# hruffieux/atlasqtl

Hardware: AMD Instinct MI355X
Metric: VB sweeps/sec (higher is better)
Workload: dtype f64; 1 GPU; atlasqtl VB sweep (S1-S22 incl. scheduled ELBO), n=1000 p=50000 q=10000, anneal=(1,2,10) on, horseshoe global-local, sweeps 6-93; n=1000, p=50000, q=10000, q_per_gpu=10000, parallelism=trait-sharded x1, env_overrides=

## Files before the change

atlasqtl_amd/csrc/aq_core_sweep.h:

```cpp
#pragma once
#include <hip/hip_runtime.h>
#include "aq_special.h"
#include "aq_plan_const.h"

typedef double aq_d4 __attribute__((ext_vector_type(4)));

struct AqCoreArgs {
  const double2 *XA;
  const double2 *XU;
  const double *G;
  const double *Gx;
  double *R;
  double *gam;
  double *mu;
  const double *Aarr;
  const double *Barr;
  const double *coef;
  const double *inv2s;
  const double *cst;
  const double *sig2b;
  double *sums;
  double *rowGB;
  double c;
  int p, q;
  int p_pad, q_pad, n_pad, nb, ntile;
  int dmode;
  int mode;
  int nseg;
  int stagger;
  int *done;
  int *errflag;
  int C;
  int xtouch;
  int xhelper;
  double *Pbuf;
  int *pflag;
  double *rnpart;
  const double *mis;
  const double *GK;
  const double *tau, *log_tau;
  const double *sig2_inv_p, *log_sig2_inv_p;
  long long *dbg;
  const double *theta;
  const double *zeta;
  double sqrt_c;
  int c_is_one;
  int mprio;
  int hprio;
};

__device__ __forceinline__ aq_d4 aq_mfma(double a, double b, aq_d4 c) {
  return __builtin_amdgcn_mfma_f64_16x16x4f64(a, b, c, 0, 0, 0);
}
__device__ __forceinline__ void aq_lds_barrier() { asm volatile("s_waitcnt lgkmcnt(0)\n\ts_barrier" ::: "memory"); }
__device__ __forceinline__ int aq_drow(int dmode, int reg, int g) { return (dmode ? 1 : 4) * reg + (dmode ? 4 : 1) * g; }
```

atlasqtl_amd/csrc/aq_core_sweep_la.h:

```cpp
#pragma once
#include <hip/hip_runtime.h>
#include "aq_core_sweep.h"
#include <type_traits>

typedef double aq_v2 __attribute__((ext_vector_type(2)));

__device__ __forceinline__ double aq_row16_sum(double v) {
  auto step = [&](auto ctrl) __attribute__((always_inline)) {
    constexpr int C = decltype(ctrl)::value;
    const int lo = __builtin_amdgcn_update_dpp(0, __double2loint(v), C, 0xf, 0xf, false);
    const int hi = __builtin_amdgcn_update_dpp(0, __double2hiint(v), C, 0xf, 0xf, false);
    v += __hiloint2double(hi, lo);
  };
  step(std::integral_constant<int, 0xB1>{});
  step(std::integral_constant<int, 0x4E>{});
  step(std::integral_constant<int, 0x124>{});
  step(std::integral_constant<int, 0x128>{});
  return v;
}

#ifndef AQ_GLDS_AUX
#define AQ_GLDS_AUX 2
#endif
__device__ __forceinline__ void aq_glds16(const void *gsrc_lane, void *lds_base) {
// ... 206 lines not shown
  }

  constexpr int NTT = 3 * (NT + NT2) + NT3;
  const int nblk_s = a.mode == 1 ? 0 : nblk;
  auto run = [&](auto ntc, auto rolec, auto hook) __attribute__((always_inline)) {
    constexpr int NTC = decltype(ntc)::value;
    constexpr int ROLE = decltype(rolec)::value;
    constexpr bool HI = ROLE == 0;
    constexpr int ST = (NTC + 2) / 3;
    const int my_t0 = part * NTT + (ROLE == 0 ? mw * NT : ROLE == 1 ? 3 * NT + (mw - 3) * NT2 : 3 * (NT + NT2));
    const int slot = ROLE == 2 ? NWM : mw;
    aq_d4 Rr[TT][NTC];
    unsigned long long mb0 = 0, mb1 = 0;
    aq_static_for<TT>([&](auto ttc) __attribute__((always_inline)) {
      constexpr int tt = decltype(ttc)::value;
      const double *Rg = a.R + (size_t)(tile0 + tt) * a.n_pad * 16 + (size_t)(16 * my_t0 + g) * 16 + col;
      aq_static_for<NTC>([&](auto tc) __attribute__((always_inline)) {
        constexpr int t = decltype(tc)::value;
#pragma unroll
        for (int r = 0; r < 4; r++) Rr[tt][t][r] = Rg[(16 * t + 4 * r) * 16];
        if constexpr (MASK) {
          const double *Mg = a.mis + (size_t)tile0 * a.n_pad * 16 + (size_t)(16 * my_t0 + g) * 16 + col;
#pragma unroll
          for (int r = 0; r < 4; r++)
            if (Mg[(16 * t + 4 * r) * 16] != 0.0) { if (t < 16) mb0 |= 1ull << (4 * (t & 15) + r); else mb1 |= 1ull << (4 * (t & 15) + r); }
        }
      });
    });
    auto remask = [&](auto tc) __attribute__((always_inline)) {
      constexpr int t = decltype(tc)::value;
      const unsigned long long mb = t < 16 ? mb0 : mb1;
#pragma unroll
      for (int r = 0; r < 4; r++) Rr[0][t][r] = ((mb >> (4 * (t & 15) + r)) & 1ull) ? Rr[0][t][r] : 0.0;
    };
    const unsigned voff = (unsigned)((my_t0 * 128 + lane) * 16);
    const char *XUb = (const char *)a.XU, *XAb = (const char *)a.XA;
    const long long BLK = (long long)NTT * C * 128 * 16;
    aq_v2 p0, p1, q0, q1, c0, c1, d0, d1;
#ifdef AQ_FORCE_DEEP_DB
#ifdef AQ_FORCE_DEEP_TT2
    constexpr bool DEEP = (NTC >= 4);
#else
    constexpr bool DEEP = (TT == 1) && (NTC >= 4);
#endif
    constexpr int DB = !DEEP ? 1 : AQ_FORCE_DEEP_DB;
#elif defined(AQ_FORCE_DEEP_MASK_DB)
    constexpr bool DEEP = (TT == 1) && (NTC >= 4) && (MASK || true);
    constexpr int DB = !DEEP ? 1 : MASK ? AQ_FORCE_DEEP_MASK_DB : (NT <= 11) ? AQ_DEEP_TT1 : 3;
#else
    constexpr bool DEEP = (TT == 1) && (NTC >= 4) && (!MASK || (SEG && NT <= 11));
    constexpr int DB = !DEEP ? 1 : (!MASK && NT <= 11) ? AQ_DEEP_TT1 : 3;
#endif
    aq_v2 xb[DB][2], ab[DB][2];
    auto dangling = [&](const char *xu0, const char *xa0, auto skip_first) __attribute__((always_inline)) {
      aq_static_for<DB - 1>([&](auto jc) __attribute__((always_inline)) {
        constexpr int j = decltype(jc)::value;
        if constexpr (!(decltype(skip_first)::value && j == 0)) {
          constexpr int kb = (j + 2) / 4, imm = (j - 4 * kb) * 2048;
          AQ_LD2I(xb[j][0], xb[j][1], voff, xu0 + kb * 8192, imm);
        }
        if constexpr (j <= DB - 3) {
          constexpr int kb = (j + 2) / 4, imm = (j - 4 * kb) * 2048;
          AQ_LD2I(ab[j][0], ab[j][1], voff, xa0 + kb * 8192, imm);
        }
      });
    };
    if constexpr (DEEP) {
      dangling(XUb + seg_b0 * BLK, XAb + seg_b0 * BLK, std::false_type{});
    } else {
      AQ_LD2(p0, p1, voff, XUb + seg_b0 * BLK);
      AQ_LD2(c0, c1, voff, XAb + seg_b0 * BLK);
    }
    for (int i = 0; i <= nblk + 1; i++) {
      const bool do_u = i >= 2, do_s = i < nblk_s;
      const double mflag = do_u ? -1.0 : 0.0;
      const int bu = seg_b0 + (i >= 2 ? i - 2 : 0), bs = seg_b0 + (i < nblk ? i : nblk - 1);
      const int nbu = seg_b0 + (i >= 1 ? (i - 1 < nblk ? i - 1 : nblk - 1) : 0), nbs = seg_b0 + (i + 1 < nblk ? i + 1 : nblk - 1);
      tl_mark(i, 0);
      hook(i);
      tl_mark(i, 1);
      if (do_u && (ROLE != 2 || a.mode == 1)) wait_ge(6, i - 1);
      if (ROLE == 1 && a.stagger) wait_ge(8 + (mw - 3), i + 1);
      tl_mark(i, 2);
      double nd[TT][4];
      {
        unsigned zero = 0;
        asm volatile("" : "+v"(zero));
        const int ln = __builtin_amdgcn_mbcnt_hi(~0u, __builtin_amdgcn_mbcnt_lo(~0u, zero));
        const double *dl = &Ldel[bu & 1][(ln >> 4) * NTR + (ln & 15)];
#pragma unroll
        for (int tt = 0; tt < TT; tt++)
#pragma unroll
          for (int s = 0; s < 4; s++) nd[tt][s] = dl[4 * NTR * s + 16 * tt] * mflag;
      }
      aq_d4 acc[TT];
#pragma unroll
      for (int tt = 0; tt < TT; tt++) acc[tt] = (aq_d4){0, 0, 0, 0};
      const char *xu = XUb + __builtin_amdgcn_readfirstlane(bu) * BLK, *xa = XAb + __builtin_amdgcn_readfirstlane(bs) * BLK;
      const char *nxu = XUb + __builtin_amdgcn_readfirstlane(nbu) * BLK, *nxa = XAb + __builtin_amdgcn_readfirstlane(nbs) * BLK;
      if (ROLE != 2 && a.mprio) __builtin_amdgcn_s_setprio(0);
      auto U = [&](auto tc, aq_v2 u0, aq_v2 u1) __attribute__((always_inline)) {
        constexpr int t = decltype(tc)::value;
        aq_static_for<TT>([&](auto ttc) __attribute__((always_inline)) {
          constexpr int tt = decltype(ttc)::value;
          aq_d4 Rt = Rr[tt][t];
          Rt = aq_mfma(u0.x, nd[tt][0], Rt);
          Rt = aq_mfma(u0.y, nd[tt][1], Rt);
          Rt = aq_mfma(u1.x, nd[tt][2], Rt);
          Rt = aq_mfma(u1.y, nd[tt][3], Rt);
          Rr[tt][t] = Rt;
        });
      };
      auto S = [&](auto tc, aq_v2 x0, aq_v2 x1) __attribute__((always_inline)) {
        constexpr int t = decltype(tc)::value;
        aq_static_for<TT>([&](auto ttc) __attribute__((always_inline)) {
          constexpr int tt = decltype(ttc)::value;
          const aq_d4 Rp = Rr[tt][t];
          acc[tt] = aq_mfma(x0.x, Rp[0], acc[tt]);
          acc[tt] = aq_mfma(x0.y, Rp[1], acc[tt]);
          acc[tt] = aq_mfma(x1.x, Rp[2], acc[tt]);
          acc[tt] = aq_mfma(x1.y, Rp[3], acc[tt]);
        });
      };
      if constexpr (DEEP) {
        aq_static_for<NTC>([&](auto tc) __attribute__((always_inline)) {
          constexpr int t = decltype(tc)::value, last = NTC - 1;
          using TP = std::integral_constant<int, (t > 0 ? t - 1 : 0)>;
          if constexpr (t + DB - 1 <= last) {
            constexpr int k = t + DB - 1, kb = (k + 2) / 4, imm = (k - 4 * kb) * 2048;
            AQ_LD2I(xb[k % DB][0], xb[k % DB][1], voff, xu + kb * 8192, imm);
          }
          if constexpr (t + DB - 2 <= last) {
            constexpr int k = t + DB - 2, kb = (k + 2) / 4, imm = (k - 4 * kb) * 2048;
            AQ_LD2I(ab[k % DB][0], ab[k % DB][1], voff, xa + kb * 8192, imm);
          }
          constexpr int issued = aq_req_issued(DB, last, t);
          aq_wait2n<2 * (issued - 1 - aq_req_index(DB, last, 0, t))>(xb[t % DB][0], xb[t % DB][1]);
          U(tc, xb[t % DB][0], xb[t % DB][1]);
          __builtin_amdgcn_sched_barrier(0);
          if constexpr (t >= 1) {
            constexpr int k = t - 1;
            aq_wait2n<2 * (issued - 1 - aq_req_index(DB, last, 1, k))>(ab[k % DB][0], ab[k % DB][1]);
            S(TP{}, ab[k % DB][0], ab[k % DB][1]);
            __builtin_amdgcn_sched_barrier(0);
          }
          if constexpr (MASK) {
            remask(tc);
            __builtin_amdgcn_sched_barrier(0);
          }
          if constexpr (t == last) {
            AQ_LD2I(xb[0][0], xb[0][1], voff, nxu, 0);
            aq_wait2n<2 * (issued - 1 - aq_req_index(DB, last, 1, last) + 1)>(ab[last % DB][0], ab[last % DB][1]);
            S(tc, ab[last % DB][0], ab[last % DB][1]);
            __builtin_amdgcn_sched_barrier(0);
            dangling(nxu, nxa, std::true_type{});
          }
          if constexpr (HI && t + 1 == ST) {
            if (a.stagger) signal(8 + mw, i + 1);
          }
          __builtin_amdgcn_sched_barrier(0);
        });
      } else if constexpr (NTC == 1) {
        using C0 = std::integral_constant<int, 0>;
        AQ_WAIT2(0, p0, p1);
        AQ_WAIT2(0, c0, c1);
        U(C0{}, p0, p1);
        if (HI && a.stagger) signal(8 + mw, i + 1);
        __builtin_amdgcn_sched_barrier(0);
        AQ_LD2(p0, p1, voff, nxu);
        if constexpr (MASK) remask(C0{});
        S(C0{}, c0, c1);
        __builtin_amdgcn_sched_barrier(0);
        AQ_LD2(c0, c1, voff, nxa);
      } else {
        aq_static_for<NTC>([&](auto tc) __attribute__((always_inline)) {
          constexpr int t = decltype(tc)::value;
          constexpr bool even = (t & 1) == 0, last = (t == NTC - 1);
          using TP = std::integral_constant<int, (t > 0 ? t - 1 : 0)>;
          if constexpr (!last) {
            constexpr int kb = (t + 1 + 2) / 4, imm = (t + 1 - 4 * kb) * 2048;
            if constexpr (even) { AQ_LD2I(q0, q1, voff, xu + kb * 8192, imm); }
            else { AQ_LD2I(p0, p1, voff, xu + kb * 8192, imm); }
          }
          if constexpr (t >= 1) {
            constexpr int kc = (t + 2) / 4, immc = (t - 4 * kc) * 2048;
            if constexpr (even) { AQ_LD2I(c0, c1, voff, xa + kc * 8192, immc); }
            else { AQ_LD2I(d0, d1, voff, xa + kc * 8192, immc); }
          }
          if constexpr (t == 0) AQ_WAIT2(4, p0, p1);
          else if constexpr (last && t == 1) AQ_WAIT2(2, q0, q1);
          else if constexpr (last) { if constexpr (even) AQ_WAIT2(4, p0, p1); else AQ_WAIT2(4, q0, q1); }
          else if constexpr (t == 1) { AQ_WAIT2(4, q0, q1); AQ_WAIT2(4, c0, c1); }
          else if constexpr (even) AQ_WAIT2(6, p0, p1);
          else AQ_WAIT2(6, q0, q1);
          if constexpr (even) U(tc, p0, p1); else U(tc, q0, q1);
          __builtin_amdgcn_sched_barrier(0);
          if constexpr (t >= 1) {
            if constexpr (last) { if constexpr (even) AQ_WAIT2(2, d0, d1); else AQ_WAIT2(2, c0, c1); }
            else if constexpr (t >= 2) { if constexpr (even) AQ_WAIT2(4, d0, d1); else AQ_WAIT2(4, c0, c1); }
            if constexpr (even) S(TP{}, d0, d1); else S(TP{}, c0, c1);
            __builtin_amdgcn_sched_barrier(0);
          }
          if constexpr (MASK) {
            remask(tc);
            __builtin_amdgcn_sched_barrier(0);
          }
          if constexpr (last) {
            AQ_LD2(p0, p1, voff, nxu);
            if constexpr (even) { AQ_WAIT2(2, c0, c1); S(tc, c0, c1); }
            else { AQ_WAIT2(2, d0, d1); S(tc, d0, d1); }
            __builtin_amdgcn_sched_barrier(0);
            AQ_LD2(c0, c1, voff, nxa);
          }
          if constexpr (HI && t + 1 == ST) {
            if (a.stagger) signal(8 + mw, i + 1);
          }
          __builtin_amdgcn_sched_barrier(0);
        });
      }
      if (ROLE != 2 && a.mprio) __builtin_amdgcn_s_setprio(2);
      if (do_s) {
        const int ps = bs & 1;
#pragma unroll
        for (int tt = 0; tt < TT; tt++)
#pragma unroll
          for (int r = 0; r < 4; r++) Sp[ps][slot][(4 * r + g) * NTR + 16 * tt + col] = acc[tt][r];
      }
      signal(ROLE == 2 ? 11 : mw, i + 1);
      tl_mark(i, 3);
    }
    if constexpr (DEEP) {
      asm volatile("s_waitcnt vmcnt(0)" ::: "memory");
      asm volatile("" : "+v"(xb[0][0]), "+v"(xb[0][1]), "+v"(ab[0][0]), "+v"(ab[0][1]));
      if constexpr (DB > 1) asm volatile("" : "+v"(xb[DB > 1 ? 1 : 0][0]), "+v"(xb[DB > 1 ? 1 : 0][1]), "+v"(ab[DB > 1 ? 1 : 0][0]), "+v"(ab[DB > 1 ? 1 : 0][1]));
      if constexpr (DB > 2) asm volatile("" : "+v"(xb[DB > 2 ? 2 : 0][0]), "+v"(xb[DB > 2 ? 2 : 0][1]), "+v"(ab[DB > 2 ? 2 : 0][0]), "+v"(ab[DB > 2 ? 2 : 0][1]));
      if constexpr (DB > 3) asm volatile("" : "+v"(xb[DB > 3 ? 3 : 0][0]), "+v"(xb[DB > 3 ? 3 : 0][1]), "+v"(ab[DB > 3 ? 3 : 0][0]), "+v"(ab[DB > 3 ? 3 : 0][1]));
    }
    else
      asm volatile("s_waitcnt vmcnt(0)" : "+v"(p0), "+v"(p1), "+v"(c0), "+v"(c1), "+v"(q0), "+v"(q1), "+v"(d0), "+v"(d1));
    unsigned zero2 = 0;
    asm volatile("" : "+v"(zero2));
    const int ln2 = __builtin_amdgcn_mbcnt_hi(~0u, __builtin_amdgcn_mbcnt_lo(~0u, zero2));
    double *Rout = a.R;
    asm volatile("" : "+s"(Rout));
    aq_static_for<TT>([&](auto ttc) __attribute__((always_inline)) {
      constexpr int tt = decltype(ttc)::value;
      double *Rg = Rout + (size_t)(tile0 + tt) * a.n_pad * 16 + (size_t)(16 * my_t0 + (ln2 >> 4)) * 16 + (ln2 & 15);
      double rn = 0.0;
      aq_static_for<NTC>([&](auto tc) __attribute__((always_inline)) {
        constexpr int t = decltype(tc)::value;
#pragma unroll
        for (int r = 0; r < 4; r++) {
          const double v = Rr[tt][t][r];
          Rg[(16 * t + 4 * r) * 16] = v;
          rn += v * v;
        }
      });
      Lrn[slot * 4 + (ln2 >> 4)][16 * tt + (ln2 & 15)] = rn;
    });
  };
  const auto no_hook = [](int) {};

  bool split_dead = false;
// ... 337 lines not shown
    double sv_g[MASK ? RPG : 1], sv_m[MASK ? RPG : 1], sv_xn[MASK ? RPG : 1], sv_th[MASK ? RPG : 1];
    auto pre_load = [&](int b) __attribute__((always_inline)) {
      const double *gk = gk_block(b);
#pragma unroll
      for (int r = 0; r < RPG; r++) {
        const size_t off = tbase + (size_t)(16 * b + hg + NG * r) * 16;
        const int jj = hg + NG * r;
        pl_g[r] = a.gam[off];
        pl_m[r] = a.mu[off];
        pl_xn[r] = gk[(jj * (jj + 1) / 2 + jj) * 16 + ht];
      }
    };
    auto stage_dma = [&](int b, int par, int b_next) __attribute__((always_inline)) {
#pragma unroll
      for (int r = 0; r < RPG; r++) {
        asm volatile("" : "+v"(pl_g[r]), "+v"(pl_m[r]), "+v"(pl_xn[r]), "+v"(th[r]) : : "memory");
        sv_g[r] = pl_g[r]; sv_m[r] = pl_m[r]; sv_xn[r] = pl_xn[r]; sv_th[r] = th[r];
      }
      gk_dma(b, par);
      if (b_next < seg_b1) { pre_load(b_next); theta_load(b_next); }
    };
    auto stage = [&](int b, int par) __attribute__((always_inline)) {
      double st_G[4], st_Gx[4], st_xn[MASK ? RPG : 1];
      if constexpr (MASK) {
#pragma unroll
        for (int r = 0; r < RPG; r++) { Lm1[par][lane + 64 * r] = sv_g[r] * sv_m[r]; st_xn[r] = sv_xn[r]; }
      } else {
#pragma unroll
        for (int r = 0; r < RPG; r++) Lm1[par][lane + 64 * r] = pg[r] * pm[r];
#pragma unroll
        for (int r = 0; r < 4; r++) {
          st_G[r] = a.G[(size_t)b * 256 + lane + 64 * r];
          const int bx = CXC ? (b + 1 < a.nb ? b + 1 : b) : b;
          st_Gx[r] = a.Gx[(size_t)bx * 256 + lane + 64 * r];
        }
      }
      double ls2r[MASK ? RPG : 1];
      if constexpr (MASK) {
#pragma unroll
        for (int r = 0; r < RPG; r++) {
          const int e = lane + 64 * r;
          const double is2 = a.c * (st_xn[r] + sig2_inv_h) * tau_k;
          const double s2 = aq_recip_pos(is2);
          const double ls2 = -aq_log_pos(is2);
          const double cf = a.c * s2 * tau_k;
          Lcoef[par][e] = cf;
          LK[par][e] = cf * cf * (a.c * 0.5 * is2);
          Ls2[par][e] = s2;
          Lls2[par][e] = ls2;
          Lxn[par][e] = st_xn[r];
          ls2r[r] = ls2;
        }
      }
      auto emitA = [&](int r, double A) __attribute__((always_inline)) {
        const int j = 16 * b + hg + NG * r, e = lane + 64 * r;
        const bool valid = kvalid && j < a.p;
        if constexpr (MASK) {
          LA[par][e] = a.c * ((valid ? A : 0.0) - 0.5 * ls2r[r] + cstna_k);
        } else {
          LA[par][e] = a.c * ((valid ? A : 0.0) + cst_k);
        }
      };
      auto emitZ = [&](int r, double zb, double za) __attribute__((always_inline)) {
        const int j = 16 * b + hg + NG * r, e = lane + 64 * r;
        const bool valid = kvalid && j < a.p;
        LB[par][e] = valid ? zb : 0.0;
        Laa[par][e] = valid ? za : 0.0;
      };
      auto emit2 = [&](int r, double A, double zb, double za) __attribute__((always_inline)) {
        const int j = 16 * b + hg + NG * r, e = lane + 64 * r;
        const bool valid = kvalid && j < a.p;
        LB[par][e] = valid ? zb : 0.0;
        Laa[par][e] = valid ? za : 0.0;
        if constexpr (MASK) LA[par][e] = a.c * ((valid ? A : 0.0) - 0.5 * Lls2[par][e] + cstna_k);
        else LA[par][e] = a.c * ((valid ? A : 0.0) + cst_k);
      };
      double uu[RPG];
      bool inr = true;
#pragma unroll
      for (int r = 0; r < RPG; r++) {
        uu[r] = (MASK ? sv_th[r] : th[r]) + zk;
        inr = inr && fabs(uu[r]) < AQ_PT_R && fabs(a.sqrt_c * uu[r]) < AQ_PT_R;
      }
      {
        constexpr int NC = AQ_PT_DEG + 1, S = AQ_PT_NI, F = NC * S;
        auto locate = [&](double x, double *xloc) __attribute__((always_inline)) {
          const double t = fmin(fabs(x) * (1.0 / AQ_PT_W), AQ_PT_NI * (1.0 - 0x1p-53));
          const int i = (int)t;
          *xloc = fma(2.0, t - (double)i, -1.0);
          return ptab + i;
        };
        {
          double co[2][NC], xl[2];
          auto fetch = [&](int r, auto setc) __attribute__((always_inline)) {
            constexpr int set = decltype(setc)::value;
            aq_lds_cdouble *pp = locate(uu[r], &xl[set]);
#pragma unroll
            for (int k = 0; k < NC; k++) co[set][k] = pp[k * S];
          };
          fetch(0, std::integral_constant<int, 0>{});
          aq_static_for<RPG>([&](auto rc) __attribute__((always_inline)) {
            constexpr int r = decltype(rc)::value, set = r & 1;
            if constexpr (r + 1 < RPG) fetch(r + 1, std::integral_constant<int, (r + 1) & 1>{});
            __builtin_amdgcn_sched_barrier(0);
            double pa = co[set][NC - 1];
#pragma unroll
            for (int k = NC - 2; k >= 0; k--) pa = fma(pa, xl[set], co[set][k]);
            emitA(r, uu[r] < 0.0 ? -pa : pa);
            __builtin_amdgcn_sched_barrier(0);
          });
        }
        {
          double co[2][2 * NC], xl[2];
          auto fetch = [&](int r, auto setc) __attribute__((always_inline)) {
            constexpr int set = decltype(setc)::value;
            aq_lds_cdouble *pp = locate(a.sqrt_c * uu[r], &xl[set]);
#pragma unroll
            for (int k = 0; k < NC; k++) {
              co[set][k] = pp[F + k * S];
              co[set][NC + k] = pp[2 * F + k * S];
            }
          };
          fetch(0, std::integral_constant<int, 0>{});
          aq_static_for<RPG>([&](auto rc) __attribute__((always_inline)) {
            constexpr int r = decltype(rc)::value, set = r & 1;
            if constexpr (r + 1 < RPG) fetch(r + 1, std::integral_constant<int, (r + 1) & 1>{});
            __builtin_amdgcn_sched_barrier(0);
            double pb = co[set][NC - 1], pd = co[set][2 * NC - 1];
#pragma unroll
            for (int k = NC - 2; k >= 0; k--) {
              pb = fma(pb, xl[set], co[set][k]);
              pd = fma(pd, xl[set], co[set][NC + k]);
            }
            const double d = uu[r] < 0.0 ? -pd : pd;
            emitZ(r, pb * inv_sqrt_c, uu[r] - 0.5 * inv_sqrt_c * (pb + d));
            __builtin_amdgcn_sched_barrier(0);
          });
        }
      }
      if (__builtin_expect(!__all(inr), 0)) {
#pragma unroll 1
        for (int r = 0; r < RPG; r++) {
          double ur = uu[0];
#pragma unroll
          for (int k = 1; k < RPG; k++) ur = (r == k) ? uu[k] : ur;
          double A, bM, dM, dummy;
          aq_probit_tab_eval<1>(ur, ptab, &A, &dummy, &dummy);
          aq_probit_tab_eval<2>(a.sqrt_c * ur, ptab, &dummy, &bM, &dM);
          emit2(r, A, bM * inv_sqrt_c, ur - 0.5 * inv_sqrt_c * (bM + dM));
        }
      }
      if constexpr (MASK) {
#ifdef AQ_DIAG_TIME
        const long long t_dma = __builtin_readcyclecounter();
#endif
        asm volatile("s_waitcnt vmcnt(0)" ::: "memory");
#ifdef AQ_DIAG_TIME
        dg_wait += __builtin_readcyclecounter() - t_dma;
#endif
      } else {
#pragma unroll
        for (int r = 0; r < 4; r++) {
          const int e = lane + 64 * r;
          LG[par][(e >> 4) * 32 + (e & 15)] = st_G[r];
          LGx[CXC ? (b + 1) % 3 : par][e] = st_Gx[r];
        }
      }
    };
    double cs0 = 0.0, cs1 = 0.0, cs2 = 0.0, cs3 = 0.0, cs5 = 0.0;
    auto finalize = [&](int b, int par) __attribute__((always_inline)) {
#pragma unroll
      for (int r = 0; r < RPG; r++) {
        const int e = lane + 64 * r, hj = hg + NG * r;
        const double gm = Lgam[par][e], mu = Lmu[par][e];
        const size_t off = tbase + (size_t)(16 * b + hj) * 16;
        if (lead) {
          a.gam[off] = gm;
          a.mu[off] = mu;
        }
        const int j = 16 * b + hj;
        double gb = 0.0;
        if (kvalid && j < a.p) {
          const double be = gm * mu;
          gb = Laa[par][e] + gm * LB[par][e];
          cs0 += gm;
          cs3 += gb;
          if constexpr (MASK) {
            const double s2 = Ls2[par][e];
            const double m2 = (mu * mu + s2) * gm;
            const double xn = Lxn[par][e];
            cs1 += m2;
            cs2 += xn * (m2 - be * be);
            cs5 += gm * Lls2[par][e];
          } else {
            cs1 += (mu * mu + sig2b_k) * gm;
            cs2 += be * be;
          }
        }
        gb = aq_row16_sum(gb);
        if ((ht & 15) == 0 && lead) a.rowGB[(size_t)(tile0 + (ht >> 4)) * a.p_pad + j] = gb;
      }
    };
    auto exchange = [&](int b) __attribute__((always_inline)) {
      const int par = b & 1, kdone = b - seg_b0 + 1;
      if constexpr (WIDE) tl_mark(kdone, 0);
#pragma unroll
      for (int m = 0; m < NWM; m++) wait_ge(m, kdone);
      if constexpr (NT3 > 0) wait_ge(11, kdone);
      if constexpr (WIDE) tl_mark(kdone, 1);
      double own[RPG];
#pragma unroll
      for (int r = 0; r < RPG; r++) {
        const int e = lane + 64 * r;
        double sv = Sp[par][0][e];
#pragma unroll
        for (int ww = 1; ww < NPS; ww++) sv += Sp[par][ww][e];
        own[r] = sv;
      }
      if constexpr (WIDE) split_exchange_wide(b, own, [] {});
      else split_exchange(b, own, [] {});
#pragma unroll
      for (int r = 0; r < RPG; r++) Stot[par][lane + 64 * r] = own[r];
      signal(14, kdone);
    };
    if (a.mode == 1) {
      for (int b = seg_b0; b < seg_b1; b++) {
        const int k = b - seg_b0, par = b & 1;
        if (k >= 2) {
#pragma unroll
          for (int m = 0; m < NWM; m++) wait_ge(m, k + 1);
          if (NT3 > 0) wait_ge(11, k + 1);
        }
#pragma unroll
        for (int r = 0; r < RPG; r++) {
          const int e = lane + 64 * r, hj = hg + NG * r;
          const size_t off = tbase + (size_t)(16 * b + hj) * 16;
          double gm = a.gam[off], mu = a.mu[off];
          double be = gm * mu;
          Ldel[par][e] = be;
          if (kvalid && (16 * b + hj) < a.p) {
            const double m2 = (mu * mu + sig2b_k) * gm;
            cs0 += gm;
            cs1 += m2;
            if constexpr (MASK) cs2 += gk_block(b)[(hj * (hj + 1) / 2 + hj) * 16 + ht] * (m2 - be * be);
            else cs2 += be * be;
          }
        }
        signal(6, k + 1);
      }
    } else {
      int xt[8] = {0, 0, 0, 0, 0, 0, 0, 0};
      const long long xt_blk = (long long)NTT * C * 2048;
      const int xt_nsl = (int)((xt_blk + 8191) / 8192);
      const int xt_wg = (int)(gridDim.x < 256 ? gridDim.x : 256) / 8 > 0 ? (int)(gridDim.x < 256 ? gridDim.x : 256) / 8 : 1;
// ... 93 lines not shown
```

atlasqtl_amd/csrc/aq_plan.h:

```cpp
#pragma once
#include <algorithm>
#include <cstdio>
#include <cstdlib>
#include <functional>
#include <string>

#include "../../include/atlasqtl_hip.h"
#include "aq_plan_const.h"

struct AqPlanInput {
  int n = 0, p = 0, q = 0;
  bool has_missing = false;
  int max_missing = 0;
  int max_short_list = 0;
  int ncu = 256;
  long long total_bytes = -1;
  const char *mem_error = nullptr;
};

struct AqPlan {
  bool use_la = false;
  bool use_mis = false;
  bool use_tw = false;
  bool la_mask = false;
  bool la_wide = false;
  int NT = 0;
  int NT2 = 0;
  int NT3x = -1;
  int TT = 1;
  int laC = 1;
  int misC = 1;
  int chain = 0;
  int stagger = 0;
  int la_xhelper = 0;
  int la_xtouch = 1;
  int la_hprio = 0;
  int la_mprio = 1;
  int NE = 0;
  int WPT = 1;
  int tw_ns = 4;
  int Mmax = 0, NR = 0;
  int p_pad = 0, q_pad = 0, n_pad = 0, nb = 0, ntile = 0;
  int ncu = 256;
};

using AqEnv = std::function<const char *(const char *)>;

enum AqHook { AQ_H_NCU, AQ_H_KERNEL, AQ_H_LA_C, AQ_H_GK_MAX_GB, AQ_H_MIS_C, AQ_H_TW_WPT, AQ_H_TT, AQ_H_NT3, AQ_H_LA_NOSPLIT,
              AQ_H_LA_XHELPER, AQ_H_XTOUCH, AQ_H_MPRIO, AQ_H_HPRIO, AQ_H_STAGGER, AQ_H_CHAIN, AQ_H_COUNT };
static const char *const aq_hook_names[AQ_H_COUNT] = {"AQ_NCU", "AQ_KERNEL", "AQ_LA_C", "AQ_GK_MAX_GB", "AQ_MIS_C", "AQ_TW_WPT", "AQ_TT", "AQ_NT3",
                                                      "AQ_LA_NOSPLIT", "AQ_LA_XHELPER", "AQ_XTOUCH", "AQ_MPRIO", "AQ_HPRIO", "AQ_STAGGER", "AQ_CHAIN"};
struct AqOpt { bool set = false, seen = false; int v = 0; double d = 0.0; };
struct AqHooks {
  const AqEnv &env;
  AqOpt opt[AQ_H_COUNT];
  const AqOpt &operator[](AqHook h) {
    AqOpt &o = opt[h];
    if (!o.seen) {
      o.seen = true;
      if (const char *v = env ? env(aq_hook_names[h]) : nullptr) { o.set = true; o.v = atoi(v); o.d = atof(v); }
    }
    return o;
  }
};

static inline int aq_plan_fail(std::string *err, int code, const std::string &msg) {
  if (err) *err = msg;
  return code;
}
static inline int aq_round16(int x) { return (x + 15) / 16 * 16; }

static inline int aq_plan_gk_budget(const AqPlanInput &in, AqHooks &h, bool wide, bool *la_mask_ok, std::string *err) {
  const size_t ntile_ = (size_t)(in.q + 15) / 16, nb_ = (size_t)(in.p + 15) / 16;
  const size_t gk_b = ntile_ * nb_ * AQ_GK_STRIDE * sizeof(double);
  const size_t rest_b = 2 * ntile_ * nb_ * 256 * sizeof(double) + 3 * (size_t)(in.n + 64) * nb_ * 16 * sizeof(double) * 2 +
                        3 * ntile_ * (size_t)(in.n + 64) * 16 * sizeof(double);
  const bool mem_known = in.total_bytes >= 0;
  if (wide && !mem_known) return aq_plan_fail(err, AQ_ERR_DEVICE, std::string("hipMemGetInfo: ") + (in.mem_error ? in.mem_error : "failed"));
  if (!mem_known || (!wide && (double)(gk_b + rest_b) * 1.05 > 0.9 * (double)in.total_bytes)) *la_mask_ok = false;
  const AqOpt &e = h[AQ_H_GK_MAX_GB];
  if (e.set && (double)gk_b > e.d * 1e9) *la_mask_ok = false;
  if (wide && !*la_mask_ok) {
    char msg[256];
    snprintf(msg, sizeof msg, "Y with missing values at n = %d: the per-trait Gram blocks need %.1f GB of device memory, which does not "
             "fit; shard the traits (fewer traits per device)", in.n, (double)gk_b / 1e9);
    return aq_plan_fail(err, AQ_ERR_UNSUPPORTED, msg);
  }
  return AQ_OK;
}

static inline int aq_plan_kernel(const AqPlanInput &in, AqHooks &h, AqPlan *pl, bool *wide_out, std::string *err) {
  const AqOpt &ek = h[AQ_H_KERNEL];
  const bool n_la_ok = in.n <= 8 * 16 * 105;
  const AqOpt &ecw = h[AQ_H_LA_C];
  const bool wide = in.n > 10240 || (ecw.set && ecw.v >= 9);
  if (wide && ecw.set && (ecw.v > AQ_LA_CMAX || (in.n > 10240 && ecw.v < 9)))
    return aq_plan_fail(err, AQ_ERR_ARG, "AQ_LA_C: the wide sample split takes 9 ... " + std::to_string(AQ_LA_CMAX) + " parts");
  if (wide && ek.set && ek.v >= 2) return aq_plan_fail(err, AQ_ERR_UNSUPPORTED, "AQ_KERNEL: only the look-ahead kernel serves n > 10240");
  bool la_mask_ok = in.has_missing && n_la_ok && in.max_missing <= AQ_MIS_MMAX && !(ek.set && ek.v >= 2);
  if (wide) la_mask_ok = in.has_missing;
  if (la_mask_ok) {
    const int rc = aq_plan_gk_budget(in, h, wide, &la_mask_ok, err);
    if (rc != AQ_OK) return rc;
  }
// ... 129 lines not shown
  }
  return best;
}

static inline double aq_plan_la_wide(AqPlan *pl, const AqOpt &ec, int ntiles) {
  auto helper_us = [](int C) { return 8.5 + 0.14 * (C - 12); };
  double best = 1e300;
  pl->la_wide = true;
  const int cf = ec.set ? ec.v : 0;
  for (int C = 9; C <= AQ_LA_CMAX && C <= pl->ncu; C++) {
    if (cf >= 9 && C != cf) continue;
    const int NT = ((ntiles + C - 1) / C + 5) / 6;
    if (NT > 18) continue;
    const double rounds = (double)(((long long)pl->ntile * C + pl->ncu - 1) / pl->ncu);
    const double cost = rounds * std::max(0.213 * 2 * NT + 1.0, helper_us(C));
    if (cost < best - 1e-9) { best = cost; pl->laC = C; pl->NT = NT; pl->NT2 = NT; pl->NT3x = -1; pl->n_pad = 16 * 6 * NT * C; }
  }
  return best;
}

static inline int aq_plan_la(const AqPlanInput &in, AqHooks &h, bool wide, AqPlan *pl, std::string *err) {
  const int ntiles = (in.n + 15) / 16;
  const bool split = !(in.n <= 1056 && !h[AQ_H_LA_C].set);
  pl->TT = (4LL * pl->ntile >= 7LL * pl->ncu) ? 2 : 1;
  const AqOpt &ett = h[AQ_H_TT];
  if (ett.set) pl->TT = ett.v == 2 ? 2 : 1;
  if (pl->la_mask) pl->TT = 1;
  if (split) pl->TT = 1;
  if (pl->TT == 2) {
    pl->q_pad = (in.q + 31) / 32 * 32;
    pl->ntile = pl->q_pad / 16;
  }
  const AqOpt &e3 = h[AQ_H_NT3];
  if (!split) {
    const int rc = aq_plan_la_unsplit(h, pl, e3, ntiles, err);
    if (rc != AQ_OK) return rc;
  } else {
    const AqOpt &ec = h[AQ_H_LA_C];
    const double best = wide ? aq_plan_la_wide(pl, ec, ntiles) : aq_plan_la_medium(pl, e3, ec, ntiles);
    if (best >= 1e300) return aq_plan_fail(err, AQ_ERR_UNSUPPORTED, "no look-ahead geometry for this n");
    pl->la_xhelper = wide ? 1 : 0;
  }
  if (h[AQ_H_LA_XHELPER].set) pl->la_xhelper = h[AQ_H_LA_XHELPER].v != 0;
  if (h[AQ_H_XTOUCH].set) pl->la_xtouch = h[AQ_H_XTOUCH].v != 0;
  if (pl->la_mask && pl->laC <= 1) pl->la_hprio = 1;
  if (pl->TT == 2 && pl->NT >= 8 && (pl->NT3x == 9 || (pl->NT3x < 0 && pl->NT2 == pl->NT - 1))) pl->la_hprio = 1;
  if (h[AQ_H_MPRIO].set) pl->la_mprio = h[AQ_H_MPRIO].v != 0;
  const AqOpt &ehp = h[AQ_H_HPRIO];
  if (ehp.set) pl->la_hprio = ehp.v >= 0 && ehp.v <= 3 ? ehp.v : 0;
  if (pl->TT == 2) pl->stagger = (pl->NT + 2) / 3;
  const AqOpt &est = h[AQ_H_STAGGER];
  if (est.set) pl->stagger = est.v >= 0 ? est.v : 0;
  pl->chain = aq_plan_chain(h, false, pl->ntile / pl->TT, pl->nb, pl->ncu, pl->laC > 1);
  if (pl->la_wide) pl->Mmax = pl->la_mask ? aq_round16(in.max_short_list) : 0;
  else if (pl->la_mask) pl->Mmax = aq_round16(in.max_missing);
  if ((pl->la_wide || pl->la_mask) && pl->Mmax < 16) pl->Mmax = 16;
  if (pl->la_mask) pl->NR = pl->n_pad + 8;
  return AQ_OK;
}

static inline int aq_plan_wide_budget(const AqPlanInput &in, const AqPlan &pl, std::string *err) {
  const double xb = 2.0 * (double)pl.nb * (pl.n_pad / 16) * 128 * sizeof(double);
  const double rb = (pl.la_mask ? 2.0 : 1.0) * (double)pl.ntile * pl.n_pad * 16 * sizeof(double);
  const double gb = pl.la_mask ? (double)pl.ntile * pl.nb * AQ_GK_STRIDE * sizeof(double) + (double)pl.nb * (pl.n_pad + 8) * 16 * sizeof(double) +
                                     (double)pl.ntile * 16 * pl.Mmax * sizeof(int)
                               : 0.0;
  if (in.total_bytes < 0) return aq_plan_fail(err, AQ_ERR_DEVICE, "hipMemGetInfo failed");
  if ((xb + rb + gb) * 1.05 > 0.9 * (double)in.total_bytes) {
    char msg[256];
    snprintf(msg, sizeof msg, "n = %d, p = %d, q = %d: the wide sample split needs %.1f GB of device memory, more than the device holds; "
             "shard the traits (fewer traits per device)", in.n, in.p, in.q, (xb + rb + gb) * 1.05 / 1e9);
    return aq_plan_fail(err, AQ_ERR_UNSUPPORTED, msg);
  }
  return AQ_OK;
}

static inline int aq_make_plan(const AqPlanInput &in, const AqEnv &env, AqPlan *out, std::string *err) {
  if (in.n > AQ_N_MAX)
    return aq_plan_fail(err, AQ_ERR_UNSUPPORTED, "n = " + std::to_string(in.n) + " exceeds the largest supported sample count, n <= " +
                                                     std::to_string(AQ_N_MAX) + " (AQ_N_MAX, the wide sample split)");
  AqHooks h{env, {}};
  AqPlan pl;
  pl.p_pad = aq_round16(in.p);
  pl.q_pad = aq_round16(in.q);
  pl.nb = pl.p_pad / 16;
  pl.ntile = pl.q_pad / 16;
  pl.ncu = in.ncu;
  if (h[AQ_H_NCU].set && h[AQ_H_NCU].v > 0) pl.ncu = h[AQ_H_NCU].v;
  bool wide = false;
  int rc = aq_plan_kernel(in, h, &pl, &wide, err);
  if (rc != AQ_OK) return rc;
  if (pl.use_mis) aq_plan_mis(in, h, &pl);
  else if (pl.use_tw) aq_plan_tw(in, h, &pl);
  else rc = aq_plan_la(in, h, wide, &pl, err);
  if (rc == AQ_OK && pl.la_wide) rc = aq_plan_wide_budget(in, pl, err);
  if (rc != AQ_OK) return rc;
  *out = pl;
  return AQ_OK;
}

static inline int aq_core_kernel_id(const AqPlan &pl) { return pl.use_mis ? 3 : pl.use_tw ? 2 : 0; }
static inline void aq_plan_to_status(const AqPlan &pl, aq_vb_status *st) {
  st->core_kernel = aq_core_kernel_id(pl);
  st->split_parts = pl.use_la ? pl.laC : pl.use_mis ? pl.misC : 1;
  st->tiles_per_group = pl.use_la ? pl.TT : 1;
  st->chain_segments = pl.chain > 1 ? pl.chain : 0;
// ... 7 lines not shown
```

atlasqtl_amd/csrc/aq_vb_sweep.hip:

```cpp
#include <hip/hip_runtime.h>

#include <cmath>
#include <cstdio>
#include <cstdlib>
#include <limits>
#include <string>
#include <vector>

#include "aq_vb.h"
#include "aq_launch_la.h"
#include "aq_sweep_kernels.h"

bool aq_all_equal_1(double c) { return std::fabs(c - 1.0) < 1.5e-8; }

static int aq_launch_tw(aq_vb *s, int mode, double c) {
  AqTwArgs &t = s->tw_args;
  t.c = c; t.mode = mode;
  size_t lds = (size_t)(s->tw_ns * s->n_pad + 8 * 256 + 32) * sizeof(double);
#define AQ_TW(NE_, WPT_)                                                                                       \
  if (s->NE == NE_ && s->WPT == WPT_) {                                                                        \
    AQ_HIP(hipFuncSetAttribute((const void *)aq_trait_wave_kernel<NE_, WPT_>, hipFuncAttributeMaxDynamicSharedMemorySize, (int)lds)); \
    hipLaunchKernelGGL((aq_trait_wave_kernel<NE_, WPT_>), dim3(s->ntile * WPT_), dim3(1024), lds, 0, t);     \
  } else
  AQ_TW(4, 1) AQ_TW(8, 1) AQ_TW(16, 1) AQ_TW(32, 1)
// ... 24 lines not shown
  if (s->misC > 1)
    hipLaunchKernelGGL(aq_k_sum_parts, dim3((s->q_pad + 255) / 256), dim3(256), 0, 0, s->rnpart.get(), s->sums.get() + (size_t)4 * s->q_pad, s->misC, s->q_pad);
  AQ_HIP(hipGetLastError());
  return AQ_OK;
}

static int aq_diag_begin(unsigned nwg, long long **dbg) {
  static AqDev<long long> *dbg_buf = new AqDev<long long>();
  static size_t dbg_cap = 0;
  const size_t dbg_n = (size_t)32 * nwg * 8 * 3 + 8 * 32 * 8;
  if (dbg_n > dbg_cap) {
    dbg_cap = 0;
    AQ_TRY(dbg_buf->alloc(dbg_n));
    dbg_cap = dbg_n;
  }
  AQ_HIP(hipMemsetAsync(dbg_buf->get(), 0, dbg_n * sizeof(long long), 0));
  *dbg = dbg_buf->get();
  return AQ_OK;
}
static int aq_diag_dump(const char *dump, const long long *dbg, unsigned grid) {
  AQ_HIP(hipDeviceSynchronize());
  std::vector<long long> h((size_t)grid * 24 + 8 * 32 * 8);
  AQ_HIP(hipMemcpy(h.data(), dbg, h.size() * sizeof(long long), hipMemcpyDeviceToHost));
  if (FILE *f = fopen(dump, "w")) {
    for (unsigned b = 0; b < grid; b++)
      for (int w = 0; w < 8; w++)
        fprintf(f, "%u %d %lld %lld %lld\n", b, w, h[((size_t)b * 8 + w) * 3], h[((size_t)b * 8 + w) * 3 + 1], h[((size_t)b * 8 + w) * 3 + 2]);
    fclose(f);
  }
  if (FILE *f = fopen((std::string(dump) + ".timeline").c_str(), "w")) {
    const long long *t = h.data() + (size_t)grid * 24;
    for (int w = 0; w < 8; w++)
      for (int i = 0; i < 32; i++)
        fprintf(f, "%d %d %lld %lld %lld %lld %lld %lld %lld\n", w, 64 + i, t[(w * 32 + i) * 8], t[(w * 32 + i) * 8 + 1], t[(w * 32 + i) * 8 + 2],
                t[(w * 32 + i) * 8 + 3], t[(w * 32 + i) * 8 + 4], t[(w * 32 + i) * 8 + 5], t[(w * 32 + i) * 8 + 6]);
    fclose(f);
  }
  return AQ_OK;
}

static int aq_launch_core(aq_vb *s, int mode, double c) {
  hipEvent_t e0, e1;
  AQ_HIP(hipEventCreate(&e0));
  AQ_HIP(hipEventCreate(&e1));
  AQ_HIP(hipEventRecord(e0, 0));
  if (s->use_mis) {
    AQ_TRY(aq_launch_mis(s, mode, c));
  } else if (s->use_tw) {
    AQ_TRY(aq_launch_tw(s, mode, c));
  } else if (s->use_la) {
    AqCoreArgs &a = s->core_args;
    a.mode = mode; a.c = c; a.sqrt_c = std::sqrt(c);
    a.c_is_one = aq_all_equal_1(c) ? 1 : 0;
    const unsigned nwg = (unsigned)(s->ntile / s->TT);
    if (s->laC > 1 && (!a.Pbuf || !a.rnpart || !a.errflag)) return aq_fail(AQ_ERR_DEVICE, "sample split without its exchange buffers");
    if (s->laC > 1 && mode == 0)
      AQ_HIP(hipMemsetAsync(s->Pbuf.get(), 0, aq_pbuf_elems(*s) * sizeof(double), 0));
    a.dbg = nullptr;
    const char *dump = getenv("AQ_DIAG_DUMP");
    if (dump && mode == 0) AQ_TRY(aq_diag_begin(nwg, &a.dbg));
    const bool chained = (mode == 0 && s->chain > 1);
    a.nseg = chained ? s->chain : 1;
    if (chained) AQ_HIP(hipMemsetAsync(s->done.get(), 0, (size_t)s->ntile * sizeof(int), 0));
    const unsigned grid = chained ? (unsigned)((long long)s->chain * nwg) : nwg * (unsigned)s->laC;
    int lrc = s->la_wide ? (s->la_mask ? aq_la_launch_wide_mask(s->NT, grid, 0, a) : aq_la_launch_wide(s->NT, grid, 0, a))
              : s->la_mask ? aq_la_launch_mask(s->NT, s->NT2, s->NT3x, chained, grid, 0, a)
              : s->TT == 2 ? aq_la_launch_tt2(s->NT, s->NT2, s->NT3x, chained, grid, 0, a) : aq_la_launch_tt1(s->NT, s->NT2, s->NT3x, chained, grid, 0, a);
    if (lrc != 0) return aq_fail(AQ_ERR_UNSUPPORTED, "no look-ahead kernel instantiation for this n");
    if (chained) {
      if (s->la_mask) hipLaunchKernelGGL(aq_k_combine_segment_sums6, dim3((s->q_pad + 255) / 256), dim3(256), 0, 0, s->sums.get(), s->q_pad, s->chain);
      else hipLaunchKernelGGL(aq_k_combine_segment_sums, dim3((s->q_pad + 255) / 256), dim3(256), 0, 0, s->sums.get(), s->q_pad, s->chain);
    }
    if (s->laC > 1)
      hipLaunchKernelGGL(aq_k_sum_parts, dim3((s->q_pad + 255) / 256), dim3(256), 0, 0, s->rnpart.get(), s->sums.get() + (size_t)4 * s->q_pad, s->laC, s->q_pad);
    if (a.dbg && s->it == 15) AQ_TRY(aq_diag_dump(dump, a.dbg, grid));
  } else {
    return aq_fail(AQ_ERR_UNSUPPORTED, "no core kernel selected for this problem");
  }
  AQ_HIP(hipEventRecord(e1, 0));
  AQ_HIP(hipGetLastError());
  if (mode == 0) {
    s->ev.push_back({e0, e1});
  } else {
    hipEventDestroy(e0);
    hipEventDestroy(e1);
  }
  return AQ_OK;
}

static int aq_launch_prepass(aq_vb *s, double c, int do_H) {
  AqPrepass &v = s->pre_args;
  v.sqrt_c = std::sqrt(c);
  v.c_is_one = aq_all_equal_1(c) ? 1 : 0;
  v.do_H = do_H;
  hipLaunchKernelGGL(aq_k_prepass, dim3(s->nHchunk, s->ntile), dim3(256), 0, 0, v);
  AQ_HIP(hipGetLastError());
  return AQ_OK;
}

static int aq_sweep_part_a(aq_vb *s) {
  if (!s->pre_done && !s->fused) AQ_TRY(aq_launch_prepass(s, s->c, 0));
  s->pre_done = false;
  hipLaunchKernelGGL(aq_k_qpre, dim3((s->q_pad + 255) / 256), dim3(256), 0, 0, s->qv, s->sc.get(), s->c);
  AQ_TRY(aq_launch_core(s, 0, s->c));
  hipLaunchKernelGGL(aq_k_reduce_rows, dim3((s->p_pad + 63) / 64), dim3(256), 0, 0, s->fused ? (const double *)nullptr : s->rowA.get(), s->rowGB.get(),
                     s->red, s->ntile, s->p_pad, s->WPT);
// ... 191 lines not shown
```

Measured before the change: 29.45 sweeps/s.

## Trim padded-sample MFMAs, edge-iteration work, and c==1 table lookups in look-ahead sweep

Adds a trim bitmask (default all on, overridable via AQ_TRIM) that enables several skip paths in the look-ahead core kernel. It skips MFMA k-steps covering padded samples in the last sample block, and skips the update/scatter MFMAs on pipeline prologue and epilogue iterations where their results are masked off. When c equals 1 it reuses the first table lookup for the second polynomial table and drops the c and sqrt(c) scaling. For tiles with no padding it removes per-element validity checks. Together these remove redundant arithmetic on padding and warm-up iterations, at the cost of more code paths, more branches inside the inner loop and some risk of divergence or register pressure.

```diff
diff --git a/atlasqtl_amd/csrc/aq_core_sweep.h b/atlasqtl_amd/csrc/aq_core_sweep.h
--- a/atlasqtl_amd/csrc/aq_core_sweep.h
+++ b/atlasqtl_amd/csrc/aq_core_sweep.h
@@ -47,6 +47,8 @@
   int c_is_one;
   int mprio;
   int hprio;
+  int ks_last;
+  int trim;
 };
 
 __device__ __forceinline__ aq_d4 aq_mfma(double a, double b, aq_d4 c) {
diff --git a/atlasqtl_amd/csrc/aq_core_sweep_la.h b/atlasqtl_amd/csrc/aq_core_sweep_la.h
--- a/atlasqtl_amd/csrc/aq_core_sweep_la.h
+++ b/atlasqtl_amd/csrc/aq_core_sweep_la.h
@@ -282,6 +282,9 @@
     constexpr int DB = !DEEP ? 1 : (!MASK && NT <= 11) ? AQ_DEEP_TT1 : 3;
 #endif
     aq_v2 xb[DB][2], ab[DB][2];
+    constexpr bool KS_ROLE = !DEEP && (NT3 > 0 ? ROLE == 2 : ROLE == 1);
+    const int ksl = KS_ROLE ? __builtin_amdgcn_readfirstlane(((ROLE == 2 || mw == NWM - 1) && part == C - 1) ? a.ks_last : 4) : 4;
+    const bool edge_trim = !DEEP && (a.trim & 2) != 0;
     auto dangling = [&](const char *xu0, const char *xa0, auto skip_first) __attribute__((always_inline)) {
       aq_static_for<DB - 1>([&](auto jc) __attribute__((always_inline)) {
         constexpr int j = decltype(jc)::value;
@@ -303,6 +306,7 @@
     }
     for (int i = 0; i <= nblk + 1; i++) {
       const bool do_u = i >= 2, do_s = i < nblk_s;
+      const bool run_u = do_u || !edge_trim, run_s = do_s || !edge_trim;
       const double mflag = do_u ? -1.0 : 0.0;
       const int bu = seg_b0 + (i >= 2 ? i - 2 : 0), bs = seg_b0 + (i < nblk ? i : nblk - 1);
       const int nbu = seg_b0 + (i >= 1 ? (i - 1 < nblk ? i - 1 : nblk - 1) : 0), nbs = seg_b0 + (i + 1 < nblk ? i + 1 : nblk - 1);
@@ -347,11 +351,23 @@
           constexpr int tt = decltype(ttc)::value;
           const aq_d4 Rp = Rr[tt][t];
           acc[tt] = aq_mfma(x0.x, Rp[0], acc[tt]);
-          acc[tt] = aq_mfma(x0.y, Rp[1], acc[tt]);
-          acc[tt] = aq_mfma(x1.x, Rp[2], acc[tt]);
-          acc[tt] = aq_mfma(x1.y, Rp[3], acc[tt]);
+          if constexpr (KS_ROLE && t == NTC - 1) {
+            if (ksl > 1) {
+              acc[tt] = aq_mfma(x0.y, Rp[1], acc[tt]);
+              if (ksl > 2) {
+                acc[tt] = aq_mfma(x1.x, Rp[2], acc[tt]);
+                if (ksl > 3) acc[tt] = aq_mfma(x1.y, Rp[3], acc[tt]);
+              }
+            }
+          } else {
+            acc[tt] = aq_mfma(x0.y, Rp[1], acc[tt]);
+            acc[tt] = aq_mfma(x1.x, Rp[2], acc[tt]);
+            acc[tt] = aq_mfma(x1.y, Rp[3], acc[tt]);
+          }
         });
       };
+      auto Ug = [&](auto tc, aq_v2 u0, aq_v2 u1) __attribute__((always_inline)) { if (run_u) U(tc, u0, u1); };
+      auto Sg = [&](auto tc, aq_v2 x0, aq_v2 x1) __attribute__((always_inline)) { if (run_s) S(tc, x0, x1); };
       if constexpr (DEEP) {
         aq_static_for<NTC>([&](auto tc) __attribute__((always_inline)) {
           constexpr int t = decltype(tc)::value, last = NTC - 1;
@@ -366,12 +382,12 @@
           }
           constexpr int issued = aq_req_issued(DB, last, t);
           aq_wait2n<2 * (issued - 1 - aq_req_index(DB, last, 0, t))>(xb[t % DB][0], xb[t % DB][1]);
-          U(tc, xb[t % DB][0], xb[t % DB][1]);
+          Ug(tc, xb[t % DB][0], xb[t % DB][1]);
           __builtin_amdgcn_sched_barrier(0);
           if constexpr (t >= 1) {
             constexpr int k = t - 1;
             aq_wait2n<2 * (issued - 1 - aq_req_index(DB, last, 1, k))>(ab[k % DB][0], ab[k % DB][1]);
-            S(TP{}, ab[k % DB][0], ab[k % DB][1]);
+            Sg(TP{}, ab[k % DB][0], ab[k % DB][1]);
             __builtin_amdgcn_sched_barrier(0);
           }
           if constexpr (MASK) {
@@ -381,7 +397,7 @@
           if constexpr (t == last) {
             AQ_LD2I(xb[0][0], xb[0][1], voff, nxu, 0);
             aq_wait2n<2 * (issued - 1 - aq_req_index(DB, last, 1, last) + 1)>(ab[last % DB][0], ab[last % DB][1]);
-            S(tc, ab[last % DB][0], ab[last % DB][1]);
+            Sg(tc, ab[last % DB][0], ab[last % DB][1]);
             __builtin_amdgcn_sched_barrier(0);
             dangling(nxu, nxa, std::true_type{});
           }
@@ -394,12 +410,12 @@
         using C0 = std::integral_constant<int, 0>;
         AQ_WAIT2(0, p0, p1);
         AQ_WAIT2(0, c0, c1);
-        U(C0{}, p0, p1);
+        Ug(C0{}, p0, p1);
         if (HI && a.stagger) signal(8 + mw, i + 1);
         __builtin_amdgcn_sched_barrier(0);
         AQ_LD2(p0, p1, voff, nxu);
         if constexpr (MASK) remask(C0{});
-        S(C0{}, c0, c1);
+        Sg(C0{}, c0, c1);
         __builtin_amdgcn_sched_barrier(0);
         AQ_LD2(c0, c1, voff, nxa);
       } else {
@@ -423,12 +439,12 @@
           else if constexpr (t == 1) { AQ_WAIT2(4, q0, q1); AQ_WAIT2(4, c0, c1); }
           else if constexpr (even) AQ_WAIT2(6, p0, p1);
           else AQ_WAIT2(6, q0, q1);
-          if constexpr (even) U(tc, p0, p1); else U(tc, q0, q1);
+          if constexpr (even) Ug(tc, p0, p1); else Ug(tc, q0, q1);
           __builtin_amdgcn_sched_barrier(0);
           if constexpr (t >= 1) {
             if constexpr (last) { if constexpr (even) AQ_WAIT2(2, d0, d1); else AQ_WAIT2(2, c0, c1); }
             else if constexpr (t >= 2) { if constexpr (even) AQ_WAIT2(4, d0, d1); else AQ_WAIT2(4, c0, c1); }
-            if constexpr (even) S(TP{}, d0, d1); else S(TP{}, c0, c1);
+            if constexpr (even) Sg(TP{}, d0, d1); else Sg(TP{}, c0, c1);
             __builtin_amdgcn_sched_barrier(0);
           }
           if constexpr (MASK) {
@@ -437,8 +453,8 @@
           }
           if constexpr (last) {
             AQ_LD2(p0, p1, voff, nxu);
-            if constexpr (even) { AQ_WAIT2(2, c0, c1); S(tc, c0, c1); }
-            else { AQ_WAIT2(2, d0, d1); S(tc, d0, d1); }
+            if constexpr (even) { AQ_WAIT2(2, c0, c1); Sg(tc, c0, c1); }
+            else { AQ_WAIT2(2, d0, d1); Sg(tc, d0, d1); }
             __builtin_amdgcn_sched_barrier(0);
             AQ_LD2(c0, c1, voff, nxa);
           }
@@ -882,18 +898,24 @@
           ls2r[r] = ls2;
         }
       }
-      auto emitA = [&](int r, double A) __attribute__((always_inline)) {
-        const int j = 16 * b + hg + NG * r, e = lane + 64 * r;
-        const bool valid = kvalid && j < a.p;
+      int hgo = hg;
+      asm volatile("" : "+v"(hgo));
+      auto emitA = [&](auto c1c, auto avc, int r, double A) __attribute__((always_inline)) {
+        constexpr bool C1 = decltype(c1c)::value, AV = decltype(avc)::value;
+        const int j = 16 * b + hgo + NG * r, e = lane + 64 * r;
+        const double Av = AV ? A : ((kvalid && j < a.p) ? A : 0.0);
         if constexpr (MASK) {
-          LA[par][e] = a.c * ((valid ? A : 0.0) - 0.5 * ls2r[r] + cstna_k);
+          const double x = Av - 0.5 * ls2r[r] + cstna_k;
+          LA[par][e] = C1 ? x : a.c * x;
         } else {
-          LA[par][e] = a.c * ((valid ? A : 0.0) + cst_k);
+          const double x = Av + cst_k;
+          LA[par][e] = C1 ? x : a.c * x;
         }
       };
-      auto emitZ = [&](int r, double zb, double za) __attribute__((always_inline)) {
-        const int j = 16 * b + hg + NG * r, e = lane + 64 * r;
-        const bool valid = kvalid && j < a.p;
+      auto emitZ = [&](auto avc, int r, double zb, double za) __attribute__((always_inline)) {
+        constexpr bool AV = decltype(avc)::value;
+        const int j = 16 * b + hgo + NG * r, e = lane + 64 * r;
+        const bool valid = AV || (kvalid && j < a.p);
         LB[par][e] = valid ? zb : 0.0;
         Laa[par][e] = valid ? za : 0.0;
       };
@@ -907,12 +929,19 @@
       };
       double uu[RPG];
       bool inr = true;
+      const bool c_one = (a.trim & 4) != 0;
+      const bool all_valid = (a.trim & 8) != 0 && 16 * b + 16 <= a.p && tile0 * 16 + NTR <= a.q;
 #pragma unroll
       for (int r = 0; r < RPG; r++) {
         uu[r] = (MASK ? sv_th[r] : th[r]) + zk;
-        inr = inr && fabs(uu[r]) < AQ_PT_R && fabs(a.sqrt_c * uu[r]) < AQ_PT_R;
-      }
-      {
+        inr = inr && fabs(uu[r]) < AQ_PT_R;
+      }
+      if (!c_one) {
+#pragma unroll
+        for (int r = 0; r < RPG; r++) inr = inr && fabs(a.sqrt_c * uu[r]) < AQ_PT_R;
+      }
+      auto tables = [&](auto c1c, auto avc) __attribute__((always_inline)) {
+        constexpr bool C1 = decltype(c1c)::value;
         constexpr int NC = AQ_PT_DEG + 1, S = AQ_PT_NI, F = NC * S;
         auto locate = [&](double x, double *xloc) __attribute__((always_inline)) {
           const double t = fmin(fabs(x) * (1.0 / AQ_PT_W), AQ_PT_NI * (1.0 - 0x1p-53));
@@ -920,11 +949,14 @@
           *xloc = fma(2.0, t - (double)i, -1.0);
           return ptab + i;
         };
+        aq_lds_cdouble *pp1[C1 ? RPG : 1];
+        double xl1[C1 ? RPG : 1];
         {
           double co[2][NC], xl[2];
           auto fetch = [&](int r, auto setc) __attribute__((always_inline)) {
             constexpr int set = decltype(setc)::value;
             aq_lds_cdouble *pp = locate(uu[r], &xl[set]);
+            if constexpr (C1) { pp1[r] = pp; xl1[r] = xl[set]; }
 #pragma unroll
             for (int k = 0; k < NC; k++) co[set][k] = pp[k * S];
           };
@@ -936,7 +968,7 @@
             double pa = co[set][NC - 1];
 #pragma unroll
             for (int k = NC - 2; k >= 0; k--) pa = fma(pa, xl[set], co[set][k]);
-            emitA(r, uu[r] < 0.0 ? -pa : pa);
+            emitA(c1c, avc, r, uu[r] < 0.0 ? -pa : pa);
             __builtin_amdgcn_sched_barrier(0);
           });
         }
@@ -944,7 +976,9 @@
           double co[2][2 * NC], xl[2];
           auto fetch = [&](int r, auto setc) __attribute__((always_inline)) {
             constexpr int set = decltype(setc)::value;
-            aq_lds_cdouble *pp = locate(a.sqrt_c * uu[r], &xl[set]);
+            aq_lds_cdouble *pp;
+            if constexpr (C1) { pp = pp1[r]; xl[set] = xl1[r]; }
+            else pp = locate(a.sqrt_c * uu[r], &xl[set]);
 #pragma unroll
             for (int k = 0; k < NC; k++) {
               co[set][k] = pp[F + k * S];
@@ -963,11 +997,14 @@
               pd = fma(pd, xl[set], co[set][NC + k]);
             }
             const double d = uu[r] < 0.0 ? -pd : pd;
-            emitZ(r, pb * inv_sqrt_c, uu[r] - 0.5 * inv_sqrt_c * (pb + d));
+            if constexpr (C1) emitZ(avc, r, pb, uu[r] - 0.5 * (pb + d));
+            else emitZ(avc, r, pb * inv_sqrt_c, uu[r] - 0.5 * inv_sqrt_c * (pb + d));
             __builtin_amdgcn_sched_barrier(0);
           });
         }
-      }
+      };
+      if (c_one && all_valid) tables(std::true_type{}, std::true_type{});
+      else tables(std::false_type{}, std::false_type{});
       if (__builtin_expect(!__all(inr), 0)) {
 #pragma unroll 1
         for (int r = 0; r < RPG; r++) {
@@ -998,7 +1035,8 @@
       }
     };
     double cs0 = 0.0, cs1 = 0.0, cs2 = 0.0, cs3 = 0.0, cs5 = 0.0;
-    auto finalize = [&](int b, int par) __attribute__((always_inline)) {
+    auto finalize_av = [&](int b, int par, auto avc) __attribute__((always_inline)) {
+      constexpr bool AV = decltype(avc)::value;
 #pragma unroll
       for (int r = 0; r < RPG; r++) {
         const int e = lane + 64 * r, hj = hg + NG * r;
@@ -1010,7 +1048,7 @@
         }
         const int j = 16 * b + hj;
         double gb = 0.0;
-        if (kvalid && j < a.p) {
+        if (AV || (kvalid && j < a.p)) {
           const double be = gm * mu;
           gb = Laa[par][e] + gm * LB[par][e];
           cs0 += gm;
@@ -1030,6 +1068,10 @@
         gb = aq_row16_sum(gb);
         if ((ht & 15) == 0 && lead) a.rowGB[(size_t)(tile0 + (ht >> 4)) * a.p_pad + j] = gb;
       }
+    };
+    auto finalize = [&](int b, int par) __attribute__((always_inline)) {
+      if ((a.trim & 8) != 0 && 16 * b + 16 <= a.p && tile0 * 16 + NTR <= a.q) finalize_av(b, par, std::true_type{});
+      else finalize_av(b, par, std::false_type{});
     };
     auto exchange = [&](int b) __attribute__((always_inline)) {
       const int par = b & 1, kdone = b - seg_b0 + 1;
diff --git a/atlasqtl_amd/csrc/aq_plan.h b/atlasqtl_amd/csrc/aq_plan.h
--- a/atlasqtl_amd/csrc/aq_plan.h
+++ b/atlasqtl_amd/csrc/aq_plan.h
@@ -36,6 +36,7 @@
   int la_xtouch = 1;
   int la_hprio = 0;
   int la_mprio = 1;
+  int la_trim = 15;
   int NE = 0;
   int WPT = 1;
   int tw_ns = 4;
@@ -47,9 +48,9 @@
 using AqEnv = std::function<const char *(const char *)>;
 
 enum AqHook { AQ_H_NCU, AQ_H_KERNEL, AQ_H_LA_C, AQ_H_GK_MAX_GB, AQ_H_MIS_C, AQ_H_TW_WPT, AQ_H_TT, AQ_H_NT3, AQ_H_LA_NOSPLIT,
-              AQ_H_LA_XHELPER, AQ_H_XTOUCH, AQ_H_MPRIO, AQ_H_HPRIO, AQ_H_STAGGER, AQ_H_CHAIN, AQ_H_COUNT };
+              AQ_H_LA_XHELPER, AQ_H_XTOUCH, AQ_H_MPRIO, AQ_H_HPRIO, AQ_H_STAGGER, AQ_H_CHAIN, AQ_H_TRIM, AQ_H_COUNT };
 static const char *const aq_hook_names[AQ_H_COUNT] = {"AQ_NCU", "AQ_KERNEL", "AQ_LA_C", "AQ_GK_MAX_GB", "AQ_MIS_C", "AQ_TW_WPT", "AQ_TT", "AQ_NT3",
-                                                      "AQ_LA_NOSPLIT", "AQ_LA_XHELPER", "AQ_XTOUCH", "AQ_MPRIO", "AQ_HPRIO", "AQ_STAGGER", "AQ_CHAIN"};
+                                                      "AQ_LA_NOSPLIT", "AQ_LA_XHELPER", "AQ_XTOUCH", "AQ_MPRIO", "AQ_HPRIO", "AQ_STAGGER", "AQ_CHAIN", "AQ_TRIM"};
 struct AqOpt { bool set = false, seen = false; int v = 0; double d = 0.0; };
 struct AqHooks {
   const AqEnv &env;
@@ -285,6 +286,7 @@
   const AqOpt &est = h[AQ_H_STAGGER];
   if (est.set) pl->stagger = est.v >= 0 ? est.v : 0;
   pl->chain = aq_plan_chain(h, false, pl->ntile / pl->TT, pl->nb, pl->ncu, pl->laC > 1);
+  if (h[AQ_H_TRIM].set) pl->la_trim = h[AQ_H_TRIM].v & 15;
   if (pl->la_wide) pl->Mmax = pl->la_mask ? aq_round16(in.max_short_list) : 0;
   else if (pl->la_mask) pl->Mmax = aq_round16(in.max_missing);
   if ((pl->la_wide || pl->la_mask) && pl->Mmax < 16) pl->Mmax = 16;
diff --git a/atlasqtl_amd/csrc/aq_vb_sweep.hip b/atlasqtl_amd/csrc/aq_vb_sweep.hip
--- a/atlasqtl_amd/csrc/aq_vb_sweep.hip
+++ b/atlasqtl_amd/csrc/aq_vb_sweep.hip
@@ -100,6 +100,9 @@
     AqCoreArgs &a = s->core_args;
     a.mode = mode; a.c = c; a.sqrt_c = std::sqrt(c);
     a.c_is_one = aq_all_equal_1(c) ? 1 : 0;
+    const int real_last = s->n - (s->n_pad - 16);
+    a.ks_last = (s->la_trim & 1) ? std::min(4, std::max(1, (real_last + 3) / 4)) : 4;
+    a.trim = (s->la_trim & (2 | 8)) | (((s->la_trim & 4) && c == 1.0) ? 4 : 0);
     const unsigned nwg = (unsigned)(s->ntile / s->TT);
     if (s->laC > 1 && (!a.Pbuf || !a.rnpart || !a.errflag)) return aq_fail(AQ_ERR_DEVICE, "sample split without its exchange buffers");
     if (s->laC > 1 && mode == 0)
```

Measured after the change: 28.34 sweeps/s. -3.8%, worse.
